# rossng/oxmpl

Hardware: AMD Instinct MI355X
Metric: RRT iterations/sec (batched problems), R^3 10k-node tree, 64-sphere field (higher is better)
Workload: dtype f64

## Files before the change

oxmpl_amd/csrc/rrt_cells.hip:

```cpp
#include "oxhip_internal.hpp"
#include "rrt_device.hpp"
#include "rrt_resident_common.hpp"
#include "lane_query_common.hpp"
#include "lane_sampler.hpp"

namespace oxhip {

#ifndef OXHIP_CELLS_BRUTE
#define OXHIP_CELLS_BRUTE 512
#endif
constexpr uint32_t kBruteMax = OXHIP_CELLS_BRUTE;
constexpr uint32_t kFlatCap = 4096;
static_assert(kBruteMax <= kFlatCap, "the flat list holds the small trees");
constexpr int kCellsWaves = 4;
constexpr uint32_t kSelfSkipMax = 4;
constexpr uint32_t kMaxSplit = 64;
constexpr int kWholeTreeUnroll = 4;
constexpr int kMaxShell = 6;
#ifndef OXHIP_CELLS_NB
#define OXHIP_CELLS_NB 4
#endif
#ifndef OXHIP_ABLATE
#define OXHIP_ABLATE 0
#endif
#ifndef OXHIP_CELLS_NB_FROZEN
#define OXHIP_CELLS_NB_FROZEN 3
#endif
#ifndef OXHIP_CELLS_FILL_X2
#define OXHIP_CELLS_FILL_X2 7ull
#endif
#ifndef OXHIP_CELLS_TAIL
#define OXHIP_CELLS_TAIL 64
#endif
#ifdef OXHIP_CELLS_DEAL_LEGACY
#define OXHIP_CELLS_DEAL_DEPTH_FROZEN 1
#define OXHIP_CELLS_DEAL_EARLY_FROZEN 0
#define OXHIP_CELLS_DEAL_MERGE_FROZEN 0
#endif
#ifndef OXHIP_CELLS_DEAL_DEPTH_FROZEN
#define OXHIP_CELLS_DEAL_DEPTH_FROZEN OXHIP_CELLS_NB_FROZEN
#endif
#ifndef OXHIP_CELLS_DEAL_EARLY_FROZEN
#define OXHIP_CELLS_DEAL_EARLY_FROZEN 1
#endif
// ... 233 lines not shown
__device__ __forceinline__ void grid_store(CellMeta& m, const CellGrid& g, uint32_t n, uint32_t mabs_bits, uint32_t lane) {
    if (lane == 0) {
#pragma unroll
        for (int k = 0; k < 3; ++k) { m.lo[k] = g.lo[k]; m.G[k] = g.G[k]; }
        m.inv_h = g.inv_h;
        m.level = g.level;
        m.regrid_at = g.regrid_at;
        m.pool_next = g.pool_next;
        m.n_grid = n;
        m.delta_node = (float)g.delta_node;
        m.mabs_bits = mabs_bits;
        m.valid = 1u;
    }
}

template <int DIM, bool STORE>
__device__ __forceinline__ void cells_sample_block(RngWindow& rng, const DevParams& p, const double* goal_c, double goal_radius, uint32_t m, uint32_t lane,
                                                   CellsWaveLds<DIM>* sh, uint32_t js) {
    sample_block64<DIM, true>(rng, p, DIM, goal_c, goal_radius, m, lane, 0u, [&](uint32_t b, const double (&q)[DIM], uint64_t pos_after) {
        if (!STORE) return;
        const uint32_t slot = (js + b) & 63u;
#pragma unroll
        for (int k = 0; k < DIM; ++k) sh->q[k][slot] = q[k];
        sh->pos_after[slot] = pos_after;
    });
}

template <int CTRL, int ROW_MASK>
__device__ __forceinline__ uint32_t dpp_scan_step(uint32_t v) {
    return v + (uint32_t)__builtin_amdgcn_update_dpp(0, (int)v, CTRL, ROW_MASK, 0xf, false);
}
__device__ __forceinline__ uint32_t wave_scan_u32(uint32_t v) {
    v = dpp_scan_step<0x111, 0xf>(v);
    v = dpp_scan_step<0x112, 0xf>(v);
    v = dpp_scan_step<0x114, 0xf>(v);
    v = dpp_scan_step<0x118, 0xf>(v);
    v = dpp_scan_step<0x142, 0xa>(v);
    v = dpp_scan_step<0x143, 0xc>(v);
    return v;
}
// ... 206 lines not shown
__host__ __device__ __forceinline__ uint64_t cells_problem_quota(uint32_t rounds, uint32_t split) {
    uint64_t sum = 0;
    for (uint32_t part = 0; part < split; ++part) sum += cells_part_quota(rounds, part, split);
    return sum;
}
#ifndef OXHIP_CELLS_PACE_BAND
#define OXHIP_CELLS_PACE_BAND OXHIP_CELLS_SKIP_COST_INV
#endif
#ifndef OXHIP_CELLS_PACE_BEHIND
#define OXHIP_CELLS_PACE_BEHIND 2
#endif
#ifndef OXHIP_CELLS_PACE_LEVEL
#define OXHIP_CELLS_PACE_LEVEL 1
#endif

#ifndef OXHIP_CELLS_WAVES_PER_EU
#define OXHIP_CELLS_WAVES_PER_EU 2
#endif
#ifndef OXHIP_CELLS_WAVES_PER_EU_FROZEN
#define OXHIP_CELLS_WAVES_PER_EU_FROZEN 3
#endif
template <int DIM, bool STAMP, bool FROZEN>
__global__ __launch_bounds__(kCellsWaves * 64, FROZEN ? OXHIP_CELLS_WAVES_PER_EU_FROZEN : OXHIP_CELLS_WAVES_PER_EU) void rrt_cells_kernel(DevParams p) {
    constexpr int D = DIM;
    __shared__ CellsShared<DIM> shared;

    const uint32_t tid = threadIdx.x;
    const uint32_t wave = uni(tid >> 6), lane = tid & 63;
    const uint32_t split = FROZEN ? p.cells_split : 1u;
    const uint32_t xcd = blockIdx.x & 7u, unit = (blockIdx.x >> 3) * (uint32_t)kCellsWaves + wave;
// ... 71 lines not shown
    uint64_t pos_start = st0.draws;
    if (split > 1) {
        const uint32_t rounds = (budget_all + 63u) / 64u;
        j_lo = cells_part_begin(rounds, part, split) * 64u;
        j_hi = cells_part_begin(rounds, part + 1u, split) * 64u;
        if (j_hi > budget_all) j_hi = budget_all;
        if (split > kSelfSkipMax) pos_start = p.cell_part_pos[(size_t)prob * kMaxSplit + part];
    }
    const uint32_t budget = j_hi - j_lo;

    const uint64_t pw = chk_lane_power(lane), pw64 = readlane_u64(pw, 63) * kFnvPrime;

    RngWindow rng;
    rng.init(sh->rng_buf, p.seed, p.first_problem_id + prob, pos_start);
    if (split > 1 && split <= kSelfSkipMax && j_lo > 0) {
        for (uint32_t r0 = 0; r0 < j_lo; r0 += 64u) cells_sample_block<DIM, false>(rng, p, goal_c, goal_radius, 64u, lane, sh, r0);
        pos_start = rng.pos;
    }
    const uint32_t pace_skipped = split > 1 && split <= kSelfSkipMax ? j_lo / 64u : 0u;
    ProblemState st = st0;
    if (split > 1) { st.checksum = 0; st.accepted = 0; st.iterations = 0; }
    uint64_t draws_done = pos_start;
    uint32_t n = st.n_nodes;
    uint32_t mabs_bits = uni(meta.mabs_bits);
    uint32_t jr = 0, js = 0;
    int32_t stop = 1;
    uint64_t n_rounds = 0, n_lanes = 0, n_amb = 0, n_expand = 0, n_cut_conflict = 0, n_tie = 0, n_memo = 0, n_forced = 0, n_regrid = 0, n_steps = 0, n_tail = 0, n_tail_pairs = 0, n_band = 0;
    uint64_t t_ph[8] = {0, 0, 0, 0, 0, 0, 0, 0}, t_pm = 0, t_c[4] = {0, 0, 0, 0}, t_cm = 0;
    uint64_t h_lanes[8] = {0, 0, 0, 0, 0, 0, 0, 0}, h_cells[8] = {0, 0, 0, 0, 0, 0, 0, 0}, h_trips[8] = {0, 0, 0, 0, 0, 0, 0, 0};
    const uint64_t t_begin = STAMP ? (uint64_t)clock64() : 0;
#define OXHIP_CPHASE(IDX) do { if (STAMP) { const uint64_t now_ = (uint64_t)clock64(); t_ph[IDX] += now_ - t_pm; t_pm = now_; } } while (0)
    uint32_t memo_n = 0xFFFFFFFFu, memo_idx = kNoNode;
    double memo_g = 0.0, memo_q[D];
#pragma unroll
    for (int k = 0; k < D; ++k) memo_q[k] = 0.0;

    while (true) {
        if (jr >= budget) { stop = 1; break; }
        if (!FROZEN && n >= p.max_nodes) { stop = 2; break; }
        if (!FROZEN && n >= grid.regrid_at) {
            cells_build<DIM>(p, prob, n, lane, c0, grid, mabs_bits);
            if (STAMP) ++n_regrid;
        }
        uint32_t m = budget - jr < 64u ? budget - jr : 64u;
        if (js < jr + m) {
            uint32_t lane_s = lane;
            if (FROZEN) asm volatile("" : "+v"(lane_s));
            cells_sample_block<DIM, true>(rng, p, goal_c, goal_radius, jr + m - js, lane_s, sh, js);
            js = jr + m;
        }
        if (STAMP) { ++n_rounds; n_lanes += m; t_pm = (uint64_t)clock64(); }
        const bool act = lane < m;
        const uint32_t slot = (jr + (act ? lane : 0u)) & 63u;
        double q[D];
#pragma unroll
        for (int k = 0; k < D; ++k) q[k] = sh->q[k][slot];
        const uint64_t pos_after_l = sh->pos_after[slot];

        Top2 t2{__builtin_inff(), __builtin_inff(), kNoNode};
        float tq[3] = {0.0f, 0.0f, 0.0f};
        uint32_t cq[3] = {0u, 0u, 0u};
#pragma unroll
        for (int k = 0; k < D; ++k) {
            tq[k] = (float)((q[k] - grid.lo[k]) * grid.inv_h);
            const float fl = floorf(tq[k]);
            uint32_t gk = grid.G[k];
            if (FROZEN) asm volatile("" : "+s"(gk));
            cq[k] = fl > 0.0f ? (fl < (float)gk ? (uint32_t)fl : grid.G[k] - 1u) : 0u;
        }
        const uint32_t gmax = grid.G[0] > grid.G[1] ? (grid.G[0] > grid.G[2] ? grid.G[0] : grid.G[2]) : (grid.G[1] > grid.G[2] ? grid.G[1] : grid.G[2]);
        const double A = sqrt((double)D) * (grid.delta_node + (double)(gmax + 8u) * 0x1p-23) * 1.01 + 1e-30;
        int verdict;
        __builtin_amdgcn_fence(__ATOMIC_RELEASE, "workgroup");
        const bool from_memo = act && memo_matches<D>(memo_n, memo_q, n, q);
        if (grid.level == 0) {
            uint32_t lane_f = lane;
            if (FROZEN) asm volatile("" : "+v"(lane_f));
            cfloat4 mine_nd = flat[lane_f < n ? lane_f : 0u];
            Top2 ta[4] = {{__builtin_inff(), __builtin_inff(), kNoNode}, {__builtin_inff(), __builtin_inff(), kNoNode},
                          {__builtin_inff(), __builtin_inff(), kNoNode}, {__builtin_inff(), __builtin_inff(), kNoNode}};
            for (uint32_t i0 = 0; i0 < n; i0 += 64) {
                const cfloat4 cur_nd = mine_nd;
                const uint32_t nx = i0 + 64u + lane;
                mine_nd = flat[nx < n ? nx : 0u];
                const uint32_t cnt = n - i0 < 64u ? n - i0 : 64u;
                for (uint32_t t = 0; t < cnt; t += 4) {
#pragma unroll
                    for (int u = 0; u < 4; ++u) {
                        const uint32_t tt = t + (uint32_t)u < cnt ? t + (uint32_t)u : cnt - 1u;
                        cfloat4 nd;
#pragma unroll
                        for (int k = 0; k < 3; ++k) nd[k] = lbits_f32((uint32_t)__builtin_amdgcn_readlane((int)lf32_bits(cur_nd[k]), (int)tt));
                        nd[3] = 0.0f;
                        const float sv = t + (uint32_t)u < cnt ? cell_s<DIM>(nd, tq) : __builtin_inff();
                        top2_push(ta[u], sv, (i0 + tt) << 16);
                    }
                }
            }
#pragma unroll
// ... 4 lines not shown
            if (STAMP) n_steps += n;
            verdict = cells_verdict(t2, __builtin_inf(), A);
            OXHIP_CPHASE(7);
        } else {
            float gap_lo[3], gap_hi[3];
#pragma unroll
            for (int k = 0; k < 3; ++k) {
                gap_lo[k] = fmaxf(tq[k] - (float)cq[k], 0.0f) * (1.0f - 0x1p-20f);
                gap_hi[k] = fmaxf((float)(cq[k] + 1u) - tq[k], 0.0f) * (1.0f - 0x1p-20f);
            }
            uint32_t done_faces = 0;
            {
                cuint4 vo[4], vf[DIM][4];
                uint32_t fc[DIM][3];
                bool fon[DIM];
                block_load(blk, act ? (cq[2] * grid.G[1] + cq[1]) * grid.G[0] + cq[0] : 0u, vo);
#pragma unroll
                for (int a = 0; a < DIM; ++a) {
                    const bool up = gap_hi[a] < gap_lo[a];
#pragma unroll
                    for (int k = 0; k < 3; ++k) fc[a][k] = cq[k] + (k == a ? (up ? 1u : 0xFFFFFFFFu) : 0u);
                    fon[a] = act && (up ? cq[a] + 1u < grid.G[a] : cq[a] > 0u);
                    done_faces |= fon[a] ? (1u << (2 * a + (up ? 1 : 0))) : 0u;
                    block_load(blk, fon[a] ? (fc[a][2] * grid.G[1] + fc[a][1]) * grid.G[0] + fc[a][0] : 0u, vf[a]);
                }
                {
                    float off[3];
#pragma unroll
                    for (int k = 0; k < 3; ++k) off[k] = ((float)cq[k] + 0x1p-17f) - tq[k];
                    const uint32_t cnt = act ? vo[0][0] : 0u;
                    block_eval<DIM>(vo, cnt < kBlkEntries ? cnt : kBlkEntries, off, t2);
                    if (__ballot(cnt > kBlkEntries) != 0) chain_follow<DIM>(blk, vo[0][1], cnt, act, off, t2);
                }
#pragma unroll
                for (int a = 0; a < DIM; ++a) {
                    float off[3];
#pragma unroll
                    for (int k = 0; k < 3; ++k) off[k] = ((float)fc[a][k] + 0x1p-17f) - tq[k];
                    const uint32_t cnt = fon[a] ? vf[a][0][0] : 0u;
                    block_eval<DIM>(vf[a], cnt < kBlkEntries ? cnt : kBlkEntries, off, t2);
                    if (__ballot(cnt > kBlkEntries) != 0) chain_follow<DIM>(blk, vf[a][0][1], cnt, fon[a], off, t2);
                }
            }
            if (STAMP) ++n_steps;
            float thr2;
            {
                const double dd = sqrt((double)t2.s1) * (1.0 + 0x1p-20) + 2.0 * A;
                thr2 = t2.s1 < __builtin_inff() ? f32_up(dd * dd * (1.0 + 0x1p-20)) : __builtin_inff();
            }
            constexpr int NO = DIM == 3 ? 26 : 8;
            constexpr uint8_t kOrder3[26] = {12, 14, 10, 16, 4, 22,  9, 11, 15, 17, 3, 5, 21, 23, 1, 7, 19, 25,  0, 2, 6, 8, 18, 20, 24, 26};
            constexpr uint8_t kOrder2[8] = {12, 14, 10, 16, 9, 11, 15, 17};
            float sq_lo[3], sq_hi[3];
#pragma unroll
            for (int k = 0; k < 3; ++k) {
                sq_lo[k] = (k < DIM && cq[k] > 0u) ? gap_lo[k] * gap_lo[k] : __builtin_inff();
                sq_hi[k] = (k < DIM && cq[k] + 1u < grid.G[k]) ? gap_hi[k] * gap_hi[k] : __builtin_inff();
            }
            auto needed = [&](float thr) -> uint32_t {
                const float th = fminf(thr, 0x1.fffffep+127f);
                uint32_t bits = 0;
#pragma unroll
                for (int b = 0; b < NO; ++b) {
                    const int o = DIM == 3 ? kOrder3[b] : kOrder2[b];
                    const int d[3] = {o % 3 - 1, (o / 3) % 3 - 1, o / 9 - 1};
                    float l = 0.0f;
                    bool first = true;
#pragma unroll
                    for (int k = 0; k < 3; ++k) {
                        if (d[k] == 0) continue;
                        const float g2 = d[k] < 0 ? sq_lo[k] : sq_hi[k];
                        l = first ? g2 : l + g2;
// ... 68 lines not shown
                            const uint32_t ow = pr & 63u;
                            float tqo[3];
                            uint32_t cqo[3], cco[3];
#pragma unroll
                            for (int k = 0; k < 3; ++k) {
                                tqo[k] = k < DIM ? lbits_f32((uint32_t)__builtin_amdgcn_ds_bpermute((int)(ow << 2), (int)lf32_bits(tq[k]))) : 0.0f;
                                cqo[k] = k < DIM ? (uint32_t)__builtin_amdgcn_ds_bpermute((int)(ow << 2), (int)cq[k]) : 0u;
                            }
                            const uint32_t o = mine[u] ? order_o(pr >> 8) : 13u;
                            const uint32_t o3 = (o * 11u) >> 5, o9 = (o3 * 11u) >> 5;
                            cco[0] = cqo[0] + (o - 3u * o3) - 1u;
                            cco[1] = cqo[1] + (o3 - 3u * o9) - 1u;
                            cco[2] = cqo[2] + o9 - 1u;
#pragma unroll
                            for (int k = 0; k < 3; ++k) offo[f][k] = ((float)cco[k] + 0x1p-17f) - tqo[k];
                            block_load(blk, mine[u] ? (cco[2] * grid.G[1] + cco[1]) * grid.G[0] + cco[0] : 0u, v[f]);
                        };
#pragma unroll
                        for (int u = 0; u < ND; ++u) mine[u] = false;
#pragma unroll
                        for (int u = 0; u < NF; ++u) fetch(u);
#pragma unroll
                        for (int u = 0; u < ND; ++u) {
                            if (u > 0 && __ballot(mine[u]) == 0) break;
                            Top2 tp{__builtin_inff(), __builtin_inff(), kNoNode};
                            const int f = u % NF;
                            const uint32_t cnt = mine[u] ? v[f][0][0] : 0u;
                            block_eval<DIM>(v[f], cnt < kBlkEntries ? cnt : kBlkEntries, offo[f], tp);
                            if (__ballot(cnt > kBlkEntries) != 0) chain_follow<DIM>(blk, v[f][0][1], cnt, mine[u], offo[f], tp);
                            if (u + NF < ND && total > 64u * (uint32_t)(u + NF)) fetch(u + NF);
                            const uint32_t kk = lane_d + 64u * (uint32_t)u;
                            if (kDealAtomic) {
                                const uint32_t ow = sh->tail_pair[mine[u] ? kk : 0u] & 63u;
                                const uint64_t pk = ((uint64_t)lf32_bits(tp.s1) << 32) | tp.i1;
                                if (mine[u]) {
                                    const uint64_t was = __hip_atomic_fetch_min(&sh->deal_best[ow], pk, __ATOMIC_RELAXED, __HIP_MEMORY_SCOPE_WAVEFRONT);
                                    const uint32_t lost = (uint32_t)((was > pk ? was : pk) >> 32), s2b = lf32_bits(tp.s2);
                                    __hip_atomic_fetch_min(&sh->tail_i1[ow], lost < s2b ? lost : s2b, __ATOMIC_RELAXED, __HIP_MEMORY_SCOPE_WAVEFRONT);
                                }
                            } else {
                                rs1[kk] = tp.s1;
                                rs2[kk] = tp.s2;
                                ri1[kk] = tp.i1;
                            }
// ... 26 lines not shown
                }
                ++trip_no;
                bool on[NB];
                uint32_t cc[NB][3], cnt[NB];
                cuint4 v[NB][4];
#pragma unroll
                for (int t = 0; t < NB; ++t) {
                    on[t] = need != 0;
                    const uint32_t b = on[t] ? (uint32_t)(__ffs((int)need) - 1) : 0u;
                    need &= need - 1u;
                    const uint32_t o = on[t] ? order_o(b) : 13u;
                    const uint32_t o3 = (o * 11u) >> 5, o9 = (o3 * 11u) >> 5;
                    cc[t][0] = cq[0] + (o - 3u * o3) - 1u;
                    cc[t][1] = cq[1] + (o3 - 3u * o9) - 1u;
                    cc[t][2] = cq[2] + o9 - 1u;
                    block_load(blk, on[t] ? (cc[t][2] * grid.G[1] + cc[t][1]) * grid.G[0] + cc[t][0] : 0u, v[t]);
                }
#pragma unroll
                for (int t = 0; t < NB; ++t) {
                    if (__ballot(on[t]) == 0) break;
                    float off[3];
#pragma unroll
                    for (int k = 0; k < 3; ++k) off[k] = ((float)cc[t][k] + 0x1p-17f) - tq[k];
                    cnt[t] = on[t] ? v[t][0][0] : 0u;
                    block_eval<DIM>(v[t], cnt[t] < kBlkEntries ? cnt[t] : kBlkEntries, off, t2);
                    if (__ballot(cnt[t] > kBlkEntries) != 0) chain_follow<DIM>(blk, v[t][0][1], cnt[t], on[t], off, t2);
                }
                if (__ballot(need != 0) != 0) {
                    const double dd = sqrt((double)t2.s1) * (1.0 + 0x1p-20) + 2.0 * A;
                    const float thr_now = t2.s1 < __builtin_inff() ? f32_up(dd * dd * (1.0 + 0x1p-20)) : __builtin_inff();
                    need &= needed(thr_now);
                }
            }
            verdict = cells_verdict(t2, block_lb<DIM>(grid, tq, cq, 1u), A);
            OXHIP_CPHASE(0);
            uint64_t needm = __ballot(act && !from_memo && verdict == 1);
            while (needm != 0) {
                const int jl = __ffsll((unsigned long long)needm) - 1;
                needm &= needm - 1;
                if (STAMP) ++n_expand;
                float tqj[3];
                uint32_t cqj[3];
#pragma unroll
                for (int k = 0; k < 3; ++k) {
                    tqj[k] = lbits_f32((uint32_t)__builtin_amdgcn_readlane((int)lf32_bits(tq[k]), jl));
                    cqj[k] = (uint32_t)__builtin_amdgcn_readlane((int)cq[k], jl);
                }
                Top2 tj{lbits_f32((uint32_t)__builtin_amdgcn_readlane((int)lf32_bits(t2.s1), jl)),
                        lbits_f32((uint32_t)__builtin_amdgcn_readlane((int)lf32_bits(t2.s2), jl)),
                        (uint32_t)__builtin_amdgcn_readlane((int)t2.i1, jl)};
                int vj = 1;
                for (uint32_t r = 2; vj == 1; ++r) {
                    if (r > (uint32_t)kMaxShell) { vj = 2; break; }
                    const uint32_t side = 2u * r + 1u, total = DIM == 3 ? side * side * side : side * side;
                    Top2 tl{__builtin_inff(), __builtin_inff(), kNoNode};
                    for (uint32_t t = lane; t < total; t += 64) {
                        const int dx = (int)(t % side) - (int)r, dy = (int)((t / side) % side) - (int)r;
                        const int dz = DIM == 3 ? (int)(t / (side * side)) - (int)r : 0;
                        const int ax = dx < 0 ? -dx : dx, ay = dy < 0 ? -dy : dy, az = dz < 0 ? -dz : dz;
                        const int cheb = ax > ay ? (ax > az ? ax : az) : (ay > az ? ay : az);
                        const int cx = (int)cqj[0] + dx, cy = (int)cqj[1] + dy, cz = (int)cqj[2] + dz;
                        if (cheb != (int)r || cx < 0 || cy < 0 || cz < 0 || cx >= (int)grid.G[0] || cy >= (int)grid.G[1] || cz >= (int)grid.G[2]) continue;
                        const uint32_t cs[3] = {(uint32_t)cx, (uint32_t)cy, (uint32_t)cz};
                        cell_visit<DIM>(blk, ((uint32_t)cz * grid.G[1] + (uint32_t)cy) * grid.G[0] + (uint32_t)cx, true, cs, tqj, tl);
                    }
                    const uint32_t m1 = wave_min_u32(lf32_bits(tl.s1));
                    const uint64_t winm = __ballot(lf32_bits(tl.s1) == m1);
                    const uint32_t m2 = __popcll(winm) >= 2 ? m1 : wave_min_u32(lf32_bits(tl.s1) == m1 ? lf32_bits(tl.s2) : lf32_bits(tl.s1));
                    const uint32_t wi = (uint32_t)__builtin_amdgcn_readlane((int)tl.i1, __ffsll((unsigned long long)winm) - 1);
                    top2_push(tj, lbits_f32(m1), wi);
                    top2_push(tj, lbits_f32(m2), kNoNode);
                    vj = cells_verdict(tj, block_lb<DIM>(grid, tqj, cqj, r), A);
                }
                if (lane == (uint32_t)jl) { t2 = tj; verdict = vj; }
            }
        }
        OXHIP_CPHASE(6);
        uint32_t nearest = (act && verdict == 0) ? t2.i1 >> 16 : kNoNode;
        double q_near[D];
        {
            const uint32_t ni = nearest == kNoNode ? 0u : nearest;
            const cdouble4 c4 = xyz[ni];
#pragma unroll
            for (int k = 0; k < D; ++k) q_near[k] = c4[k];
        }
        double g = nearest == kNoNode ? __builtin_inf() : dist2<D>(q_near, q, DIM);
        bool clear = nearest != kNoNode && fabs(sqrt(g) * grid.inv_h - sqrt((double)t2.s1)) <= A + sqrt((double)t2.s1) * 0x1p-19 + 1e-30;
        if (p.dbg_flags & OXHIP_DEBUG_ALL_WHOLE_TREE) clear = false;
        uint64_t pace_seen = 0;
        auto pace_report = [&]() {
            const uint32_t now = pace_skipped + (uint32_t)(((uint64_t)jr * OXHIP_CELLS_SKIP_COST_INV) >> 6);
            uint32_t zv = 0;
            asm volatile("" : "+v"(zv));
            if (lane == 0) pace_seen = __hip_atomic_fetch_add(pace_ctr + zv, (uint64_t)(now - pace_sent), __ATOMIC_RELAXED, __HIP_MEMORY_SCOPE_AGENT);
            pace_sent = now;
        };
        auto pace_apply = [&]() {
            if ((p.dbg_flags & OXHIP_DEBUG_CELLS_NO_PACING) != 0) return;
            uint32_t seen_lo = (uint32_t)pace_seen, seen_hi = (uint32_t)(pace_seen >> 32);
            asm volatile("" : "+v"(seen_lo), "+v"(seen_hi));
            const uint64_t seen = ((uint64_t)uni(seen_hi) << 32) | uni(seen_lo);
            const uint64_t mean = (seen >> p.cells_quota_shift) * pace_quota, own = (uint64_t)pace_sent * pace_xcd;
            const uint64_t band = (uint64_t)OXHIP_CELLS_PACE_BAND * pace_xcd;
            if (own + band < mean) __builtin_amdgcn_s_setprio(OXHIP_CELLS_PACE_BEHIND);
            else if (own > mean + band) __builtin_amdgcn_s_setprio(0);
            else __builtin_amdgcn_s_setprio(OXHIP_CELLS_PACE_LEVEL);
        };
        if constexpr (FROZEN) pace_report();
        if (from_memo) {
            nearest = memo_idx;
            g = memo_g;
            const cdouble4 m4 = xyz[memo_idx];
#pragma unroll
            for (int k = 0; k < D; ++k) q_near[k] = m4[k];
            clear = true;
        }
        if (STAMP) n_memo += (uint64_t)__popcll(__ballot(from_memo));
        const bool amb = act && !clear;
        if (FROZEN && __ballot(amb) != 0) sh->tail_s2[lane] = (verdict == 2 && grid.level != 0) ? t2.s1 : __builtin_inff();
        const uint32_t hb = hi32(g) + 1;
        double qn[D], mid[D];
        steer<DIM>(p, false, g, q_near, q, qn);
        bool dup = g == 0.0;
        OXHIP_CPHASE(1);
        float Qf[D];
        double bb = 0.0;
#pragma unroll
        for (int k = 0; k < D; ++k) {
            const float bk = (float)(q[k] - c0[k]);
            Qf[k] = -2.0f * bk;
            bb += (double)bk * (double)bk;
        }
        bool bad = false;
        if (nobs > 0) {
            uint32_t kz = 0;
            asm volatile("" : "+v"(kz));
            double kc0[D];
            float ksg_inv[D], ksg_bias[D];
#pragma unroll
            for (int k = 0; k < D; ++k) { kc0[k] = shared.k.c0[kz + k]; ksg_inv[k] = shared.k.sg_inv[kz + k]; ksg_bias[k] = shared.k.sg_bias[kz + k]; }
            lerp<DIM>(q_near, qn, 0.5, mid, DIM);
            uint64_t cand;
            {
                const float gs = (float)p.sph_grid_G;
                bool inside = mg.usable && !(OXHIP_ABLATE & 1);
                uint32_t ci[3] = {0u, 0u, 0u};
#pragma unroll
                for (int k = 0; k < D; ++k) {
                    const float u = __builtin_fmaf((float)(mid[k] - kc0[k]), ksg_inv[k], ksg_bias[k]);
                    inside = inside && u >= -0x1p-10f && u <= gs + 0x1p-10f;
                    const float fl = floorf(u);
                    ci[k] = fl > 0.0f ? (fl < gs ? (uint32_t)fl : p.sph_grid_G - 1u) : 0u;
                }
                const uint64_t m = p.sph_grid[D == 3 ? (ci[2] * p.sph_grid_G + ci[1]) * p.sph_grid_G + ci[0] : ci[1] * p.sph_grid_G + ci[0]];
                cand = inside ? m : ~0ull;
            }
            if constexpr (FROZEN) pace_apply();
            if (ns64 < 64) cand &= (1ull << ns64) - 1ull;
            const uint64_t maybe = spheres_maybe_hit<D>(shared.obs, cand, mid);
            OXHIP_CPHASE(2);
            const bool need = !(OXHIP_ABLATE & 4) && act && !amb && (maybe != 0 || extras);
            bad = motion_own_lane_short<D>(p, shared.obs, shared.steps, need, maybe, q_near, qn, ns64, nobs);
        } else {
            if constexpr (FROZEN) pace_apply();
        }
        OXHIP_CPHASE(3);
        bool ok = act && !bad;
        constexpr bool ins = !FROZEN;
        float nf_a[D], nf_cc;
        node_f32<D>(qn, c0, nf_a, nf_cc);

        uint32_t cut = m;
        int32_t stop_after = -1;
        const uint64_t ambm = __ballot(amb);
        if (!FROZEN && ambm != 0) cut = (uint32_t)(__ffsll((unsigned long long)ambm) - 1);
        const uint32_t amb_at = cut;
        uint64_t okm = __ballot(ok && !(FROZEN && amb));
// ... 101 lines not shown
                    }
                }
                if (lane == c) confl = 0;
            }
            hitm = __ballot(hit);
            const uint64_t capm = __ballot(act && n + (uint32_t)__popcll(okm & below_mask(lane)) >= p.max_nodes);
            if (capm != 0) {
                const uint32_t c = (uint32_t)(__ffsll((unsigned long long)capm) - 1);
                if (c <= cut) { cut = c; stop_after = 2; }
            }
            if (p.stop_at_goal && hitm != 0) {
                const uint32_t c = (uint32_t)__ffsll((unsigned long long)hitm);
                if (c <= cut) { cut = c; stop_after = 0; }
            }
        }
        if ((p.dbg_flags & OXHIP_DEBUG_ONE_LANE_ROUNDS) != 0 && cut > 1) { cut = 1; stop_after = -1; if (STAMP) ++n_forced; }
        OXHIP_CPHASE(4);
        if (STAMP) t_cm = (uint64_t)clock64();
        if (cut > 0) {
            const uint64_t cutm = first_n_mask(cut);
            const bool mine = lane < cut;
            uint32_t ins_cell = 0, ins_slot = 0;
            uint64_t ins_entry = 0;
            bool ins_link = false;
            if (ins) {
                const uint32_t idx = n + (uint32_t)__popcll(okm & below_mask(lane));
                if (mine && ok) {
#pragma unroll
                    for (int k = 0; k < D; ++k) tree[(size_t)k * cap + idx] = qn[k];
                    xyz[idx] = cdouble4{qn[0], qn[1], D >= 3 ? qn[D - 1] : 0.0, 0.0};
                    parent[idx] = (int32_t)nearest;
// ... 30 lines not shown
            if (ins && grid.level != 0) {
                if (STAMP) { const uint64_t nw = (uint64_t)clock64(); t_c[0] += nw - t_cm; t_cm = nw; }
                cells_insert_finish(blk, grid.pool_next, ins_cell, ins_entry, ins_link, ins_slot, lane);
                if (STAMP) { const uint64_t nw = (uint64_t)clock64(); t_c[1] += nw - t_cm; t_cm = nw; }
            }
            st.iterations += cut;
            st.accepted += (uint64_t)__popcll(okm & cutm);
            draws_done = readlane_u64(pos_after_l, (int)(cut - 1u));
            jr += cut;
        }
        if (STAMP) { const uint64_t nw = (uint64_t)clock64(); t_c[3] += nw - t_cm; t_cm = nw; }
        OXHIP_CPHASE(5);
        if (stop_after >= 0) { stop = stop_after; break; }
        if (FROZEN ? (ambm & first_n_mask(cut)) == 0 : (cut == m || ambm == 0 || (uint32_t)(__ffsll((unsigned long long)ambm) - 1) != cut)) continue;

        if (!FROZEN && n >= p.max_nodes) { stop = 2; break; }
        uint64_t todo = FROZEN ? (ambm & first_n_mask(cut)) : 1ull;
        const uint32_t jr0 = FROZEN ? jr - cut : jr;
        bool goal_stop = false;
        const bool keep_memo = !(FROZEN && (p.dbg_flags & OXHIP_DEBUG_SHORT_MEMO) != 0);
        do {
            const uint32_t ja = FROZEN ? (uint32_t)(__ffsll((unsigned long long)todo) - 1) : 0u;
            todo &= todo - 1;
            if (STAMP) ++n_amb;
            const uint32_t slot1 = (jr0 + ja) & 63u;
            double q1[D];
#pragma unroll
            for (int k = 0; k < D; ++k) q1[k] = unid(sh->q[k][slot1]);
            const bool same_q = memo_matches<D>(memo_n, memo_q, n, q1);
            double gmin = memo_g;
// ... 278 lines not shown
```

Measured before the change: 7.431 billion.

## Outline rare frozen-path sampling and ambiguity settling, reload params from kernargs

Moves the rare sequential sampling fallback and the frozen-tree ambiguous-lane settle loop into noinline device functions. Inside the hot round loop, grid metadata, table pointers and scalar params are reloaded from the kernarg segment instead of being held live. The aim is to cut register pressure and code size in the main frozen kernel loop so occupancy or scheduling improves. The cost is extra call overhead and scalar reloads on each round, and the outlined calls may spill or perform worse on the rare paths.

```diff
diff --git a/oxmpl_amd/csrc/rrt_cells.hip b/oxmpl_amd/csrc/rrt_cells.hip
--- a/oxmpl_amd/csrc/rrt_cells.hip
+++ b/oxmpl_amd/csrc/rrt_cells.hip
@@ -28,6 +28,9 @@
 #endif
 #ifndef OXHIP_CELLS_FILL_X2
 #define OXHIP_CELLS_FILL_X2 7ull
+#endif
+#ifndef OXHIP_CELLS_OUTLINE_RARE
+#define OXHIP_CELLS_OUTLINE_RARE 1
 #endif
 #ifndef OXHIP_CELLS_TAIL
 #define OXHIP_CELLS_TAIL 64
@@ -291,16 +294,61 @@
     }
 }
 
+typedef const __attribute__((address_space(4))) DevParams* cells_kernarg_ptr;
+struct CellsSeqPos { uint64_t pos, base_blk; };
+__device__ __forceinline__ cells_kernarg_ptr cells_kernargs() { return (cells_kernarg_ptr)__builtin_amdgcn_kernarg_segment_ptr(); }
+__device__ __forceinline__ const DevParams& cells_args_at(cells_kernarg_ptr k) {
+    return *(const DevParams*)(cells_kernarg_ptr)(uintptr_t)uni64((uint64_t)(uintptr_t)k);
+}
 template <int DIM, bool STORE>
+__device__ __noinline__ CellsSeqPos cells_sample_seq(cells_kernarg_ptr kargs, __attribute__((address_space(3))) CellsWaveLds<DIM>* shl, uint32_t prob,
+                                                     uint64_t pos, uint64_t base_blk, uint32_t m, uint32_t js) {
+    const DevParams& r = cells_args_at(kargs);
+    CellsWaveLds<DIM>* sh = (CellsWaveLds<DIM>*)shl;
+    const uint32_t lane = threadIdx.x & 63u;
+    RngWindow rng;
+    rng.buf = sh->rng_buf;
+    rng.seed = r.seed;
+    rng.stream = r.first_problem_id + prob;
+    rng.pos = pos;
+    rng.base_blk = base_blk;
+    double goal_c[DIM];
+#pragma unroll
+    for (int k = 0; k < DIM; ++k) goal_c[k] = r.goal_c[(size_t)prob * DIM + k];
+    const double goal_radius = r.goal_r[prob];
+    for (uint32_t b = 0; b < m; ++b) {
+        double q[DIM];
+        sample_state<DIM, false>(rng, r, DIM, goal_c, q, goal_radius);
+        if (STORE && lane == 0) {
+            const uint32_t slot = (js + b) & 63u;
+#pragma unroll
+            for (int k = 0; k < DIM; ++k) sh->q[k][slot] = q[k];
+            sh->pos_after[slot] = rng.pos;
+        }
+    }
+    return CellsSeqPos{rng.pos, rng.base_blk};
+}
+template <int DIM, bool STORE, bool OUTLINED = false>
 __device__ __forceinline__ void cells_sample_block(RngWindow& rng, const DevParams& p, const double* goal_c, double goal_radius, uint32_t m, uint32_t lane,
-                                                   CellsWaveLds<DIM>* sh, uint32_t js) {
-    sample_block64<DIM, true>(rng, p, DIM, goal_c, goal_radius, m, lane, 0u, [&](uint32_t b, const double (&q)[DIM], uint64_t pos_after) {
+                                                   CellsWaveLds<DIM>* sh, uint32_t js, uint32_t prob = 0u) {
+    auto store = [&](uint32_t b, const double (&q)[DIM], uint64_t pos_after) {
         if (!STORE) return;
         const uint32_t slot = (js + b) & 63u;
 #pragma unroll
         for (int k = 0; k < DIM; ++k) sh->q[k][slot] = q[k];
         sh->pos_after[slot] = pos_after;
-    });
+    };
+    if constexpr (OUTLINED) {
+        rng_window_hold(rng, (uint64_t)m * (1u + (uint32_t)DIM), lane);
+        if (!sample_lanes64<DIM, true>(rng, p, DIM, goal_c, goal_radius, m, lane, store)) {
+            const CellsSeqPos e = cells_sample_seq<DIM, STORE>(cells_kernargs(), (__attribute__((address_space(3))) CellsWaveLds<DIM>*)sh, prob, rng.pos,
+                                                               rng.base_blk, m, js);
+            rng.pos = uni64(e.pos);
+            rng.base_blk = uni64(e.base_blk);
+        }
+    } else {
+        sample_block64<DIM, true>(rng, p, DIM, goal_c, goal_radius, m, lane, 0u, store);
+    }
 }
 
 template <int CTRL, int ROW_MASK>
@@ -537,6 +585,114 @@
 #define OXHIP_CELLS_PACE_LEVEL 1
 #endif
 
+template <bool FROZEN>
+__device__ __forceinline__ const DevParams& round_args(const DevParams& p) {
+    if constexpr (FROZEN) {
+        cells_kernarg_ptr k = cells_kernargs();
+        asm volatile("" : "+s"(k));
+        return *(const DevParams*)k;
+    } else {
+        return p;
+    }
+}
+
+typedef const __attribute__((address_space(4))) CellMeta* cells_meta_kptr;
+typedef const __attribute__((address_space(4))) double* cells_f64_kptr;
+template <int DIM>
+__device__ __forceinline__ void grid_load_scalar(const DevParams& r, uint32_t prob, CellGrid& g) {
+    const cells_meta_kptr m = (cells_meta_kptr)(uintptr_t)(r.cell_meta + prob);
+#pragma unroll
+    for (int k = 0; k < 3; ++k) {
+        g.lo[k] = m->lo[k];
+        g.G[k] = m->G[k];
+    }
+    g.inv_h = m->inv_h;
+    g.level = m->level;
+    g.regrid_at = m->regrid_at;
+    g.pool_next = m->pool_next;
+    g.delta_node = (double)m->delta_node;
+}
+
+struct CellsSettled {
+    uint64_t chk;
+    uint32_t accepted, memo_n, memo_idx;
+    double memo_g, memo_q[3];
+};
+template <int DIM>
+__device__ __noinline__ CellsSettled cells_settle_frozen(cells_kernarg_ptr kargs, __attribute__((address_space(3))) CellsShared<DIM>* shl, uint32_t wave,
+                                                         uint32_t prob, uint32_t n, uint64_t todo, uint32_t jr0, uint32_t cut, double A, uint32_t memo_n,
+                                                         uint32_t memo_idx, double memo_g, double mq0, double mq1, double mq2) {
+    constexpr int D = DIM;
+    const DevParams& p = cells_args_at(kargs);
+    CellsShared<DIM>& shared = *(CellsShared<DIM>*)shl;
+    CellsWaveLds<DIM>* sh = &shared.w[wave];
+    const uint32_t lane = threadIdx.x & 63u;
+    const size_t cap = p.cap;
+    const double* tree = p.tree + (size_t)prob * DIM * cap;
+    const uint8_t* skip = p.skip + (size_t)prob * cap;
+    const CellBlock* blk = p.cell_blk + (size_t)prob * p.cell_blocks;
+    const cdouble4* xyz = reinterpret_cast<const cdouble4*>(p.cell_xyz) + (size_t)prob * cap;
+    CellGrid grid;
+    grid_load_scalar<DIM>(p, prob, grid);
+    const uint32_t ns64 = p.n_spheres < 64 ? p.n_spheres : 64;
+    const bool extras = p.n_spheres + p.n_boxes > ns64;
+    const uint64_t pw = chk_lane_power(lane);
+    double memo_q[D];
+    memo_q[0] = mq0;
+    memo_q[1] = mq1;
+    if (D >= 3) memo_q[D - 1] = mq2;
+    CellsSettled out{0, 0, 0, 0, 0.0, {0.0, 0.0, 0.0}};
+    const bool keep_memo = (p.dbg_flags & OXHIP_DEBUG_SHORT_MEMO) == 0;
+    do {
+        const uint32_t ja = (uint32_t)(__ffsll((unsigned long long)todo) - 1);
+        todo &= todo - 1;
+        const uint32_t slot1 = (jr0 + ja) & 63u;
+        double q1[D];
+#pragma unroll
+        for (int k = 0; k < D; ++k) q1[k] = unid(sh->q[k][slot1]);
+        const bool same_q = memo_matches<D>(memo_n, memo_q, n, q1);
+        double gmin = memo_g;
+        uint32_t memo_hit_idx = memo_idx;
+        bool tie = false, banded = false;
+        if (!same_q && (p.dbg_flags & OXHIP_DEBUG_ALL_WHOLE_TREE) == 0) {
+            const float s1j = lbits_f32(uni(lf32_bits(sh->tail_s2[ja])));
+            banded = cells_band_resolve<DIM>(grid, blk, xyz, sh, lane, q1, s1j, A, memo_hit_idx, gmin);
+            if (banded && keep_memo) memo_keep<D>(memo_n, memo_q, memo_g, memo_idx, n, q1, gmin, memo_hit_idx);
+        }
+        if (!same_q && !banded) {
+            tie = whole_tree_nearest<D, 2>(tree, skip, cap, n, lane, q1, gmin, memo_hit_idx);
+            if (!tie && keep_memo) memo_keep<D>(memo_n, memo_q, memo_g, memo_idx, n, q1, gmin, memo_hit_idx);
+        }
+        uint32_t nearest1;
+        double qn1[D], q_near1[D];
+        if (!tie) {
+            nearest1 = memo_hit_idx;
+#pragma unroll
+            for (int k = 0; k < D; ++k) q_near1[k] = unid(tree[(size_t)k * cap + nearest1]);
+            steer<DIM>(p, false, gmin, q_near1, q1, qn1);
+        } else {
+            const double dist1 = literal_nearest<D>(tree, cap, n, lane, q1, nearest1, q_near1);
+            steer<DIM>(p, true, dist1, q_near1, q1, qn1);
+        }
+        bool ok1 = true;
+        if (p.n_spheres + p.n_boxes > 0) {
+            double oc[D];
+#pragma unroll
+            for (int k = 0; k < D; ++k) oc[k] = shared.obs[k][lane];
+            ok1 = motion_wave<D>(p, lane, q_near1, qn1, oc, shared.obs[D][lane], shared.obs[D + 1][lane], ns64, extras);
+        }
+        const uint64_t pe = readlane_u64(pw, (int)(cut - 1u - ja));
+        out.chk = uni64(out.chk + iter_digest<D>(nearest1, qn1, DIM, ok1) * pe);
+        if (ok1) out.accepted++;
+    } while (todo != 0);
+    out.memo_n = memo_n;
+    out.memo_idx = memo_idx;
+    out.memo_g = memo_g;
+#pragma unroll
+    for (int k = 0; k < D; ++k) out.memo_q[k] = memo_q[k];
+    return out;
+}
+
 #ifndef OXHIP_CELLS_WAVES_PER_EU
 #define OXHIP_CELLS_WAVES_PER_EU 2
 #endif
@@ -638,7 +794,7 @@
     RngWindow rng;
     rng.init(sh->rng_buf, p.seed, p.first_problem_id + prob, pos_start);
     if (split > 1 && split <= kSelfSkipMax && j_lo > 0) {
-        for (uint32_t r0 = 0; r0 < j_lo; r0 += 64u) cells_sample_block<DIM, false>(rng, p, goal_c, goal_radius, 64u, lane, sh, r0);
+        for (uint32_t r0 = 0; r0 < j_lo; r0 += 64u) cells_sample_block<DIM, false, FROZEN && OXHIP_CELLS_OUTLINE_RARE != 0>(rng, p, goal_c, goal_radius, 64u, lane, sh, r0, prob);
         pos_start = rng.pos;
     }
     const uint32_t pace_skipped = split > 1 && split <= kSelfSkipMax ? j_lo / 64u : 0u;
@@ -659,6 +815,22 @@
 #pragma unroll
     for (int k = 0; k < D; ++k) memo_q[k] = 0.0;
 
+    auto r_blk = [&]() -> CellBlock* {
+        if constexpr (FROZEN) { const DevParams& r = round_args<true>(p); return r.cell_blk + (size_t)prob * r.cell_blocks; } else return blk;
+    };
+    auto r_xyz = [&]() -> cdouble4* {
+        if constexpr (FROZEN) { const DevParams& r = round_args<true>(p); return reinterpret_cast<cdouble4*>(r.cell_xyz) + (size_t)prob * r.cap; } else return xyz;
+    };
+    auto r_flat = [&]() -> cfloat4* {
+        if constexpr (FROZEN) { const DevParams& r = round_args<true>(p); return reinterpret_cast<cfloat4*>(r.cell_flat) + (size_t)prob * kFlatCap; } else return flat;
+    };
+    auto cells_A = [](const CellGrid& grid) -> double {
+        const uint32_t gmax = grid.G[0] > grid.G[1] ? (grid.G[0] > grid.G[2] ? grid.G[0] : grid.G[2]) : (grid.G[1] > grid.G[2] ? grid.G[1] : grid.G[2]);
+        const double A = sqrt((double)D) * (grid.delta_node + (double)(gmax + 8u) * 0x1p-23) * 1.01 + 1e-30;
+        return A;
+    };
+    const double A_frozen = FROZEN ? unid(cells_A(grid)) : 0.0;
+
     while (true) {
         if (jr >= budget) { stop = 1; break; }
         if (!FROZEN && n >= p.max_nodes) { stop = 2; break; }
@@ -670,7 +842,19 @@
         if (js < jr + m) {
             uint32_t lane_s = lane;
             if (FROZEN) asm volatile("" : "+v"(lane_s));
-            cells_sample_block<DIM, true>(rng, p, goal_c, goal_radius, jr + m - js, lane_s, sh, js);
+            if constexpr (FROZEN) {
+                const DevParams& r = round_args<true>(p);
+                const cells_f64_kptr gk = (cells_f64_kptr)(uintptr_t)(r.goal_c + (size_t)prob * DIM);
+                double gc[D];
+#pragma unroll
+                for (int k = 0; k < D; ++k) gc[k] = gk[k];
+                const double gr = D == 2 ? ((cells_f64_kptr)(uintptr_t)r.goal_r)[prob] : 0.0;
+                rng.seed = r.seed;
+                rng.stream = r.first_problem_id + prob;
+                cells_sample_block<DIM, true, OXHIP_CELLS_OUTLINE_RARE != 0>(rng, r, gc, gr, jr + m - js, lane_s, sh, js, prob);
+            } else {
+                cells_sample_block<DIM, true>(rng, p, goal_c, goal_radius, jr + m - js, lane_s, sh, js);
+            }
             js = jr + m;
         }
         if (STAMP) { ++n_rounds; n_lanes += m; t_pm = (uint64_t)clock64(); }
@@ -684,29 +868,33 @@
         Top2 t2{__builtin_inff(), __builtin_inff(), kNoNode};
         float tq[3] = {0.0f, 0.0f, 0.0f};
         uint32_t cq[3] = {0u, 0u, 0u};
+        CellGrid grid_w;
+        if constexpr (FROZEN) grid_load_scalar<DIM>(round_args<true>(p), prob, grid_w);
+        const CellGrid& gw = *(FROZEN ? &grid_w : &grid);
+        CellBlock* const blk_w = r_blk();
 #pragma unroll
         for (int k = 0; k < D; ++k) {
-            tq[k] = (float)((q[k] - grid.lo[k]) * grid.inv_h);
+            tq[k] = (float)((q[k] - gw.lo[k]) * gw.inv_h);
             const float fl = floorf(tq[k]);
-            uint32_t gk = grid.G[k];
+            uint32_t gk = gw.G[k];
             if (FROZEN) asm volatile("" : "+s"(gk));
-            cq[k] = fl > 0.0f ? (fl < (float)gk ? (uint32_t)fl : grid.G[k] - 1u) : 0u;
-        }
-        const uint32_t gmax = grid.G[0] > grid.G[1] ? (grid.G[0] > grid.G[2] ? grid.G[0] : grid.G[2]) : (grid.G[1] > grid.G[2] ? grid.G[1] : grid.G[2]);
-        const double A = sqrt((double)D) * (grid.delta_node + (double)(gmax + 8u) * 0x1p-23) * 1.01 + 1e-30;
+            cq[k] = fl > 0.0f ? (fl < (float)gk ? (uint32_t)fl : gw.G[k] - 1u) : 0u;
+        }
+        const double A = FROZEN ? A_frozen : cells_A(grid);
         int verdict;
         __builtin_amdgcn_fence(__ATOMIC_RELEASE, "workgroup");
         const bool from_memo = act && memo_matches<D>(memo_n, memo_q, n, q);
-        if (grid.level == 0) {
+        if (gw.level == 0) {
             uint32_t lane_f = lane;
             if (FROZEN) asm volatile("" : "+v"(lane_f));
-            cfloat4 mine_nd = flat[lane_f < n ? lane_f : 0u];
+            const cfloat4* const flat_w = r_flat();
+            cfloat4 mine_nd = flat_w[lane_f < n ? lane_f : 0u];
             Top2 ta[4] = {{__builtin_inff(), __builtin_inff(), kNoNode}, {__builtin_inff(), __builtin_inff(), kNoNode},
                           {__builtin_inff(), __builtin_inff(), kNoNode}, {__builtin_inff(), __builtin_inff(), kNoNode}};
             for (uint32_t i0 = 0; i0 < n; i0 += 64) {
                 const cfloat4 cur_nd = mine_nd;
                 const uint32_t nx = i0 + 64u + lane;
-                mine_nd = flat[nx < n ? nx : 0u];
+                mine_nd = flat_w[nx < n ? nx : 0u];
                 const uint32_t cnt = n - i0 < 64u ? n - i0 : 64u;
                 for (uint32_t t = 0; t < cnt; t += 4) {
 #pragma unroll
@@ -741,15 +929,15 @@
                 cuint4 vo[4], vf[DIM][4];
                 uint32_t fc[DIM][3];
                 bool fon[DIM];
-                block_load(blk, act ? (cq[2] * grid.G[1] + cq[1]) * grid.G[0] + cq[0] : 0u, vo);
+                block_load(blk_w, act ? (cq[2] * gw.G[1] + cq[1]) * gw.G[0] + cq[0] : 0u, vo);
 #pragma unroll
                 for (int a = 0; a < DIM; ++a) {
                     const bool up = gap_hi[a] < gap_lo[a];
 #pragma unroll
                     for (int k = 0; k < 3; ++k) fc[a][k] = cq[k] + (k == a ? (up ? 1u : 0xFFFFFFFFu) : 0u);
-                    fon[a] = act && (up ? cq[a] + 1u < grid.G[a] : cq[a] > 0u);
+                    fon[a] = act && (up ? cq[a] + 1u < gw.G[a] : cq[a] > 0u);
                     done_faces |= fon[a] ? (1u << (2 * a + (up ? 1 : 0))) : 0u;
-                    block_load(blk, fon[a] ? (fc[a][2] * grid.G[1] + fc[a][1]) * grid.G[0] + fc[a][0] : 0u, vf[a]);
+                    block_load(blk_w, fon[a] ? (fc[a][2] * gw.G[1] + fc[a][1]) * gw.G[0] + fc[a][0] : 0u, vf[a]);
                 }
                 {
                     float off[3];
@@ -757,7 +945,7 @@
                     for (int k = 0; k < 3; ++k) off[k] = ((float)cq[k] + 0x1p-17f) - tq[k];
                     const uint32_t cnt = act ? vo[0][0] : 0u;
                     block_eval<DIM>(vo, cnt < kBlkEntries ? cnt : kBlkEntries, off, t2);
-                    if (__ballot(cnt > kBlkEntries) != 0) chain_follow<DIM>(blk, vo[0][1], cnt, act, off, t2);
+                    if (__ballot(cnt > kBlkEntries) != 0) chain_follow<DIM>(blk_w, vo[0][1], cnt, act, off, t2);
                 }
 #pragma unroll
                 for (int a = 0; a < DIM; ++a) {
@@ -766,7 +954,7 @@
                     for (int k = 0; k < 3; ++k) off[k] = ((float)fc[a][k] + 0x1p-17f) - tq[k];
                     const uint32_t cnt = fon[a] ? vf[a][0][0] : 0u;
                     block_eval<DIM>(vf[a], cnt < kBlkEntries ? cnt : kBlkEntries, off, t2);
-                    if (__ballot(cnt > kBlkEntries) != 0) chain_follow<DIM>(blk, vf[a][0][1], cnt, fon[a], off, t2);
+                    if (__ballot(cnt > kBlkEntries) != 0) chain_follow<DIM>(blk_w, vf[a][0][1], cnt, fon[a], off, t2);
                 }
             }
             if (STAMP) ++n_steps;
@@ -782,7 +970,7 @@
 #pragma unroll
             for (int k = 0; k < 3; ++k) {
                 sq_lo[k] = (k < DIM && cq[k] > 0u) ? gap_lo[k] * gap_lo[k] : __builtin_inff();
-                sq_hi[k] = (k < DIM && cq[k] + 1u < grid.G[k]) ? gap_hi[k] * gap_hi[k] : __builtin_inff();
+                sq_hi[k] = (k < DIM && cq[k] + 1u < gw.G[k]) ? gap_hi[k] * gap_hi[k] : __builtin_inff();
             }
             auto needed = [&](float thr) -> uint32_t {
                 const float th = fminf(thr, 0x1.fffffep+127f);
@@ -881,7 +1069,7 @@
                             cco[2] = cqo[2] + o9 - 1u;
 #pragma unroll
                             for (int k = 0; k < 3; ++k) offo[f][k] = ((float)cco[k] + 0x1p-17f) - tqo[k];
-                            block_load(blk, mine[u] ? (cco[2] * grid.G[1] + cco[1]) * grid.G[0] + cco[0] : 0u, v[f]);
+                            block_load(blk_w, mine[u] ? (cco[2] * gw.G[1] + cco[1]) * gw.G[0] + cco[0] : 0u, v[f]);
                         };
 #pragma unroll
                         for (int u = 0; u < ND; ++u) mine[u] = false;
@@ -894,7 +1082,7 @@
                             const int f = u % NF;
                             const uint32_t cnt = mine[u] ? v[f][0][0] : 0u;
                             block_eval<DIM>(v[f], cnt < kBlkEntries ? cnt : kBlkEntries, offo[f], tp);
-                            if (__ballot(cnt > kBlkEntries) != 0) chain_follow<DIM>(blk, v[f][0][1], cnt, mine[u], offo[f], tp);
+                            if (__ballot(cnt > kBlkEntries) != 0) chain_follow<DIM>(blk_w, v[f][0][1], cnt, mine[u], offo[f], tp);
                             if (u + NF < ND && total > 64u * (uint32_t)(u + NF)) fetch(u + NF);
                             const uint32_t kk = lane_d + 64u * (uint32_t)u;
                             if (kDealAtomic) {
@@ -951,7 +1139,7 @@
                     cc[t][0] = cq[0] + (o - 3u * o3) - 1u;
                     cc[t][1] = cq[1] + (o3 - 3u * o9) - 1u;
                     cc[t][2] = cq[2] + o9 - 1u;
-                    block_load(blk, on[t] ? (cc[t][2] * grid.G[1] + cc[t][1]) * grid.G[0] + cc[t][0] : 0u, v[t]);
+                    block_load(blk_w, on[t] ? (cc[t][2] * gw.G[1] + cc[t][1]) * gw.G[0] + cc[t][0] : 0u, v[t]);
                 }
 #pragma unroll
                 for (int t = 0; t < NB; ++t) {
@@ -961,7 +1149,7 @@
                     for (int k = 0; k < 3; ++k) off[k] = ((float)cc[t][k] + 0x1p-17f) - tq[k];
                     cnt[t] = on[t] ? v[t][0][0] : 0u;
                     block_eval<DIM>(v[t], cnt[t] < kBlkEntries ? cnt[t] : kBlkEntries, off, t2);
-                    if (__ballot(cnt[t] > kBlkEntries) != 0) chain_follow<DIM>(blk, v[t][0][1], cnt[t], on[t], off, t2);
+                    if (__ballot(cnt[t] > kBlkEntries) != 0) chain_follow<DIM>(blk_w, v[t][0][1], cnt[t], on[t], off, t2);
                 }
                 if (__ballot(need != 0) != 0) {
                     const double dd = sqrt((double)t2.s1) * (1.0 + 0x1p-20) + 2.0 * A;
@@ -969,7 +1157,7 @@
                     need &= needed(thr_now);
                 }
             }
-            verdict = cells_verdict(t2, block_lb<DIM>(grid, tq, cq, 1u), A);
+            verdict = cells_verdict(t2, block_lb<DIM>(gw, tq, cq, 1u), A);
             OXHIP_CPHASE(0);
             uint64_t needm = __ballot(act && !from_memo && verdict == 1);
             while (needm != 0) {
@@ -997,9 +1185,9 @@
                         const int ax = dx < 0 ? -dx : dx, ay = dy < 0 ? -dy : dy, az = dz < 0 ? -dz : dz;
                         const int cheb = ax > ay ? (ax > az ? ax : az) : (ay > az ? ay : az);
                         const int cx = (int)cqj[0] + dx, cy = (int)cqj[1] + dy, cz = (int)cqj[2] + dz;
-                        if (cheb != (int)r || cx < 0 || cy < 0 || cz < 0 || cx >= (int)grid.G[0] || cy >= (int)grid.G[1] || cz >= (int)grid.G[2]) continue;
+                        if (cheb != (int)r || cx < 0 || cy < 0 || cz < 0 || cx >= (int)gw.G[0] || cy >= (int)gw.G[1] || cz >= (int)gw.G[2]) continue;
                         const uint32_t cs[3] = {(uint32_t)cx, (uint32_t)cy, (uint32_t)cz};
-                        cell_visit<DIM>(blk, ((uint32_t)cz * grid.G[1] + (uint32_t)cy) * grid.G[0] + (uint32_t)cx, true, cs, tqj, tl);
+                        cell_visit<DIM>(blk_w, ((uint32_t)cz * gw.G[1] + (uint32_t)cy) * gw.G[0] + (uint32_t)cx, true, cs, tqj, tl);
                     }
                     const uint32_t m1 = wave_min_u32(lf32_bits(tl.s1));
                     const uint64_t winm = __ballot(lf32_bits(tl.s1) == m1);
@@ -1007,7 +1195,7 @@
                     const uint32_t wi = (uint32_t)__builtin_amdgcn_readlane((int)tl.i1, __ffsll((unsigned long long)winm) - 1);
                     top2_push(tj, lbits_f32(m1), wi);
                     top2_push(tj, lbits_f32(m2), kNoNode);
-                    vj = cells_verdict(tj, block_lb<DIM>(grid, tqj, cqj, r), A);
+                    vj = cells_verdict(tj, block_lb<DIM>(gw, tqj, cqj, r), A);
                 }
                 if (lane == (uint32_t)jl) { t2 = tj; verdict = vj; }
             }
@@ -1017,27 +1205,33 @@
         double q_near[D];
         {
             const uint32_t ni = nearest == kNoNode ? 0u : nearest;
-            const cdouble4 c4 = xyz[ni];
+            const cdouble4 c4 = r_xyz()[ni];
 #pragma unroll
             for (int k = 0; k < D; ++k) q_near[k] = c4[k];
         }
         double g = nearest == kNoNode ? __builtin_inf() : dist2<D>(q_near, q, DIM);
-        bool clear = nearest != kNoNode && fabs(sqrt(g) * grid.inv_h - sqrt((double)t2.s1)) <= A + sqrt((double)t2.s1) * 0x1p-19 + 1e-30;
-        if (p.dbg_flags & OXHIP_DEBUG_ALL_WHOLE_TREE) clear = false;
+        CellGrid grid_c;
+        if constexpr (FROZEN) grid_load_scalar<DIM>(round_args<true>(p), prob, grid_c);
+        const CellGrid& gc = *(FROZEN ? &grid_c : &grid);
+        bool clear = nearest != kNoNode && fabs(sqrt(g) * gc.inv_h - sqrt((double)t2.s1)) <= A + sqrt((double)t2.s1) * 0x1p-19 + 1e-30;
+        const DevParams& ps = round_args<FROZEN>(p);
+        if (ps.dbg_flags & OXHIP_DEBUG_ALL_WHOLE_TREE) clear = false;
         uint64_t pace_seen = 0;
         auto pace_report = [&]() {
             const uint32_t now = pace_skipped + (uint32_t)(((uint64_t)jr * OXHIP_CELLS_SKIP_COST_INV) >> 6);
             uint32_t zv = 0;
             asm volatile("" : "+v"(zv));
-            if (lane == 0) pace_seen = __hip_atomic_fetch_add(pace_ctr + zv, (uint64_t)(now - pace_sent), __ATOMIC_RELAXED, __HIP_MEMORY_SCOPE_AGENT);
+            uint64_t* const ctr = ps.cell_board + (size_t)(ps.cells_parity & 1u) * kCellsBoardWords + (size_t)xcd * (kCellsBoardWords / 8u);
+            if (lane == 0) pace_seen = __hip_atomic_fetch_add(ctr + zv, (uint64_t)(now - pace_sent), __ATOMIC_RELAXED, __HIP_MEMORY_SCOPE_AGENT);
             pace_sent = now;
         };
         auto pace_apply = [&]() {
-            if ((p.dbg_flags & OXHIP_DEBUG_CELLS_NO_PACING) != 0) return;
+            const DevParams& pp = round_args<FROZEN>(p);
+            if ((pp.dbg_flags & OXHIP_DEBUG_CELLS_NO_PACING) != 0) return;
             uint32_t seen_lo = (uint32_t)pace_seen, seen_hi = (uint32_t)(pace_seen >> 32);
             asm volatile("" : "+v"(seen_lo), "+v"(seen_hi));
             const uint64_t seen = ((uint64_t)uni(seen_hi) << 32) | uni(seen_lo);
-            const uint64_t mean = (seen >> p.cells_quota_shift) * pace_quota, own = (uint64_t)pace_sent * pace_xcd;
+            const uint64_t mean = (seen >> pp.cells_quota_shift) * pace_quota, own = (uint64_t)pace_sent * pace_xcd;
             const uint64_t band = (uint64_t)OXHIP_CELLS_PACE_BAND * pace_xcd;
             if (own + band < mean) __builtin_amdgcn_s_setprio(OXHIP_CELLS_PACE_BEHIND);
             else if (own > mean + band) __builtin_amdgcn_s_setprio(0);
@@ -1047,17 +1241,17 @@
         if (from_memo) {
             nearest = memo_idx;
             g = memo_g;
-            const cdouble4 m4 = xyz[memo_idx];
+            const cdouble4 m4 = r_xyz()[memo_idx];
 #pragma unroll
             for (int k = 0; k < D; ++k) q_near[k] = m4[k];
             clear = true;
         }
         if (STAMP) n_memo += (uint64_t)__popcll(__ballot(from_memo));
         const bool amb = act && !clear;
-        if (FROZEN && __ballot(amb) != 0) sh->tail_s2[lane] = (verdict == 2 && grid.level != 0) ? t2.s1 : __builtin_inff();
+        if (FROZEN && __ballot(amb) != 0) sh->tail_s2[lane] = (verdict == 2 && gc.level != 0) ? t2.s1 : __builtin_inff();
         const uint32_t hb = hi32(g) + 1;
         double qn[D], mid[D];
-        steer<DIM>(p, false, g, q_near, q, qn);
+        steer<DIM>(ps, false, g, q_near, q, qn);
         bool dup = g == 0.0;
         OXHIP_CPHASE(1);
         float Qf[D];
@@ -1079,7 +1273,9 @@
             lerp<DIM>(q_near, qn, 0.5, mid, DIM);
             uint64_t cand;
             {
-                const float gs = (float)p.sph_grid_G;
+                const DevParams& pf = round_args<FROZEN>(p);
+                const uint32_t sgG = pf.sph_grid_G;
+                const float gs = (float)sgG;
                 bool inside = mg.usable && !(OXHIP_ABLATE & 1);
                 uint32_t ci[3] = {0u, 0u, 0u};
 #pragma unroll
@@ -1087,9 +1283,9 @@
                     const float u = __builtin_fmaf((float)(mid[k] - kc0[k]), ksg_inv[k], ksg_bias[k]);
                     inside = inside && u >= -0x1p-10f && u <= gs + 0x1p-10f;
                     const float fl = floorf(u);
-                    ci[k] = fl > 0.0f ? (fl < gs ? (uint32_t)fl : p.sph_grid_G - 1u) : 0u;
-                }
-                const uint64_t m = p.sph_grid[D == 3 ? (ci[2] * p.sph_grid_G + ci[1]) * p.sph_grid_G + ci[0] : ci[1] * p.sph_grid_G + ci[0]];
+                    ci[k] = fl > 0.0f ? (fl < gs ? (uint32_t)fl : sgG - 1u) : 0u;
+                }
+                const uint64_t m = pf.sph_grid[D == 3 ? (ci[2] * sgG + ci[1]) * sgG + ci[0] : ci[1] * sgG + ci[0]];
                 cand = inside ? m : ~0ull;
             }
             if constexpr (FROZEN) pace_apply();
@@ -1097,7 +1293,7 @@
             const uint64_t maybe = spheres_maybe_hit<D>(shared.obs, cand, mid);
             OXHIP_CPHASE(2);
             const bool need = !(OXHIP_ABLATE & 4) && act && !amb && (maybe != 0 || extras);
-            bad = motion_own_lane_short<D>(p, shared.obs, shared.steps, need, maybe, q_near, qn, ns64, nobs);
+            bad = motion_own_lane_short<D>(round_args<FROZEN>(p), shared.obs, shared.steps, need, maybe, q_near, qn, ns64, nobs);
         } else {
             if constexpr (FROZEN) pace_apply();
         }
@@ -1229,7 +1425,7 @@
                 if (c <= cut) { cut = c; stop_after = 0; }
             }
         }
-        if ((p.dbg_flags & OXHIP_DEBUG_ONE_LANE_ROUNDS) != 0 && cut > 1) { cut = 1; stop_after = -1; if (STAMP) ++n_forced; }
+        if ((ps.dbg_flags & OXHIP_DEBUG_ONE_LANE_ROUNDS) != 0 && cut > 1) { cut = 1; stop_after = -1; if (STAMP) ++n_forced; }
         OXHIP_CPHASE(4);
         if (STAMP) t_cm = (uint64_t)clock64();
         if (cut > 0) {
@@ -1290,6 +1486,18 @@
         if (stop_after >= 0) { stop = stop_after; break; }
         if (FROZEN ? (ambm & first_n_mask(cut)) == 0 : (cut == m || ambm == 0 || (uint32_t)(__ffsll((unsigned long long)ambm) - 1) != cut)) continue;
 
+        if constexpr (FROZEN && !STAMP && DIM == 3 && OXHIP_CELLS_OUTLINE_RARE != 0) {
+            const CellsSettled r = cells_settle_frozen<DIM>(cells_kernargs(), (__attribute__((address_space(3))) CellsShared<DIM>*)&shared, wave, prob, n,
+                                                            ambm & first_n_mask(cut), jr - cut, cut, A, memo_n, memo_idx, memo_g, memo_q[0], memo_q[1], D >= 3 ? memo_q[D - 1] : 0.0);
+            st.checksum = uni64(st.checksum + r.chk);
+            st.accepted += uni(r.accepted);
+            memo_n = uni(r.memo_n);
+            memo_idx = uni(r.memo_idx);
+            memo_g = unid(r.memo_g);
+#pragma unroll
+            for (int k = 0; k < D; ++k) memo_q[k] = unid(r.memo_q[k]);
+            continue;
+        }
         if (!FROZEN && n >= p.max_nodes) { stop = 2; break; }
         uint64_t todo = FROZEN ? (ambm & first_n_mask(cut)) : 1ull;
         const uint32_t jr0 = FROZEN ? jr - cut : jr;
```

After: 7.574 billion, median of 3. About the same (+1.9%).
